# merlresearch/MC-PILCO

Hardware: NVIDIA B200
Metric: particle-steps/s (rollout fwd+bwd) (higher is better)
Workload: dtype f64

## Files before the change

### mc-pilco_b200/csrc/mcp_dgemm_tma.cu

```cuda
#include <cuda.h>

#include "mcp_dgemm.cuh"

namespace mcp {

constexpr int T_BM = 128, T_BN = 128, T_BK = 16, T_STAGES = 6, T_GROUP = 12;
constexpr int T_TILE_BYTES = T_BM * T_BK * 8;
constexpr int T_STAGE_BYTES = 2 * T_TILE_BYTES;
constexpr int T_CONSUMER_WARPS = 8;
constexpr int T_THREADS = 32 * T_CONSUMER_WARPS;
constexpr int T_LOOKAHEAD = T_STAGES - 2;
constexpr size_t T_SMEM_BYTES = (size_t)T_STAGES * T_STAGE_BYTES + 2 * T_STAGES * 8 + 1024;

__device__ __forceinline__ unsigned smem_u32(const void* p) { return (unsigned)__cvta_generic_to_shared(p); }
__device__ __forceinline__ void mbar_init(unsigned bar, unsigned count) {
  asm volatile("mbarrier.init.shared::cta.b64 [%0], %1;" ::"r"(bar), "r"(count));
}
__device__ __forceinline__ void mbar_expect_tx(unsigned bar, unsigned bytes) {
  asm volatile("mbarrier.arrive.expect_tx.shared::cta.b64 _, [%0], %1;" ::"r"(bar), "r"(bytes) : "memory");
}
__device__ __forceinline__ void mbar_arrive(unsigned bar) {
  asm volatile("mbarrier.arrive.shared::cta.b64 _, [%0];" ::"r"(bar) : "memory");
}
__device__ __forceinline__ void mbar_wait(unsigned bar, unsigned parity) {
  asm volatile(
      "{\n"
      ".reg .pred p;\n"
      "WAIT_%=:\n"
      "mbarrier.try_wait.parity.shared::cta.b64 p, [%0], %1;\n"
      "@p bra DONE_%=;\n"
      "bra WAIT_%=;\n"
      "DONE_%=:\n"
      "}\n" ::"r"(bar),
      "r"(parity)
      : "memory");
}
__device__ __forceinline__ void tma_load_2d(unsigned dst, const CUtensorMap* map, int c0, int c1, unsigned bar) {
  asm volatile("cp.async.bulk.tensor.2d.shared::cluster.global.mbarrier::complete_tx::bytes [%0], [%1, {%2, %3}], [%4];" ::"r"(dst),
               "l"(map), "r"(c0), "r"(c1), "r"(bar)
               : "memory");
}

template <bool TRIM>
__global__ void __launch_bounds__(T_THREADS, 1)
dgemm_tma_kernel(const __grid_constant__ CUtensorMap tmA, const __grid_constant__ CUtensorMap tmB, int M, int N, int K, double alpha,
                 double* __restrict__ C, int ldc, double beta, int tri, int kflags) {
  extern __shared__ unsigned char smem_raw[];
  const unsigned base = (smem_u32(smem_raw) + 1023u) & ~1023u;
  const unsigned char* tiles = smem_raw + (base - smem_u32(smem_raw));
  const unsigned bars = base + T_STAGES * T_STAGE_BYTES;
  const int warp = threadIdx.x >> 5, lane = threadIdx.x & 31;
  const int tiles_m = (M + T_BM - 1) / T_BM, tiles_n = (N + T_BN - 1) / T_BN;
  const int per_group = T_GROUP * tiles_n, group = blockIdx.x / per_group, first_m = group * T_GROUP;
  const int rows_here = min(tiles_m - first_m, T_GROUP), in_group = blockIdx.x - group * per_group;
  int mt = first_m + in_group % rows_here;
  if (TRIM && (kflags & KF_A_LOWER) && !(kflags & (KF_A_UPPER | KF_B_UPPER | KF_B_LOWER))) mt = tiles_m - 1 - mt;
  const int m0 = mt * T_BM;
  int nt = in_group / rows_here;
  if (TRIM && (kflags & KF_B_LOWER) && !(kflags & (KF_A_UPPER | KF_B_UPPER))) nt = tiles_n - 1 - nt;
  const int n0 = nt * T_BN;
  int kb = 0, ke = K;
  if (TRIM) {
    if (tri == 1 && n0 > m0 + T_BM - 1) return;
    if (kflags & KF_A_UPPER) kb = max(kb, m0);
    if (kflags & KF_B_UPPER) kb = max(kb, n0);
    if (kflags & KF_A_LOWER) ke = min(ke, m0 + T_BM);
    if (kflags & KF_B_LOWER) ke = min(ke, n0 + T_BN);
    kb = (kb / T_BK) * T_BK;
  }
  const int KT = ke > kb ? (ke - kb + T_BK - 1) / T_BK : 0;

  if (threadIdx.x == 0) {
#pragma unroll
    for (int s = 0; s < T_STAGES; s++) {
      mbar_init(bars + 8 * s, 1);
      mbar_init(bars + 8 * (T_STAGES + s), T_CONSUMER_WARPS);
    }
    asm volatile("fence.mbarrier_init.release.cluster;" ::: "memory");
  }
  __syncthreads();

  auto produce = [&](int kn) {
    const int s = kn % T_STAGES;
    if (kn >= T_STAGES) mbar_wait(bars + 8 * (T_STAGES + s), ((kn / T_STAGES) - 1) & 1);
    const unsigned full = bars + 8 * s, dst = base + s * T_STAGE_BYTES;
    mbar_expect_tx(full, T_STAGE_BYTES);
    tma_load_2d(dst, &tmA, kb + kn * T_BK, m0, full);
    tma_load_2d(dst + T_TILE_BYTES, &tmB, kb + kn * T_BK, n0, full);
  };
  if (threadIdx.x == 0) {
    asm volatile("prefetch.tensormap [%0];" ::"l"(&tmA) : "memory");
    asm volatile("prefetch.tensormap [%0];" ::"l"(&tmB) : "memory");
    for (int kn = 0; kn < T_LOOKAHEAD && kn < KT; kn++) produce(kn);
  }

  constexpr int MI = 4, NJ = 8;
  const int g = lane >> 2, q = lane & 3;
  const int wm0 = (warp & 3) * 32, wn0 = (warp >> 2) * 64;
  const unsigned kx = (unsigned)(g & 3) << 5;
  const unsigned laneE = ((unsigned)(q >> 1) << 4) | ((unsigned)(q & 1) << 3);
  const unsigned laneO = ((unsigned)((q >> 1) ^ 1) << 4) | ((unsigned)(q & 1) << 3);
  const unsigned aE = (unsigned)(wm0 + 2 * g) * 128u + laneE, aO = (unsigned)(wm0 + 2 * g + 1) * 128u + laneO;
  const unsigned bE = T_TILE_BYTES + (unsigned)(wn0 + 2 * g) * 128u + laneE, bO = T_TILE_BYTES + (unsigned)(wn0 + 2 * g + 1) * 128u + laneO;

  double acc[MI][NJ][2];
#pragma unroll
  for (int i = 0; i < MI; i++)
#pragma unroll
    for (int j = 0; j < NJ; j++) acc[i][j][0] = acc[i][j][1] = 0.0;

  for (int kt = 0; kt < KT; kt++) {
    const int s = kt % T_STAGES;
    if (threadIdx.x == 0 && kt + T_LOOKAHEAD < KT) produce(kt + T_LOOKAHEAD);
    mbar_wait(bars + 8 * s, (kt / T_STAGES) & 1);
    const unsigned char* st = tiles + s * T_STAGE_BYTES;
#pragma unroll
    for (int ks = 0; ks < T_BK / 4; ks++) {
      const unsigned ko = ((unsigned)(ks * 2) << 4) ^ kx;
      double a[MI], b[NJ];
#pragma unroll
      for (int i = 0; i < MI; i++) a[i] = *reinterpret_cast<const double*>(st + (((i & 1) ? aO : aE) + ko + (unsigned)(i >> 1) * 2048u));
#pragma unroll
      for (int j = 0; j < NJ; j++) b[j] = *reinterpret_cast<const double*>(st + (((j & 1) ? bO : bE) + ko + (unsigned)(j >> 1) * 2048u));
#pragma unroll
      for (int i = 0; i < MI; i++)
#pragma unroll
        for (int j = 0; j < NJ; j++) dmma884(acc[i][j][0], acc[i][j][1], a[i], b[j]);
    }
    __syncwarp();
    if (lane == 0) mbar_arrive(bars + 8 * (T_STAGES + s));
  }

#pragma unroll
  for (int i = 0; i < MI; i++) {
    const int r = m0 + wm0 + 16 * (i >> 1) + 2 * g + (i & 1);
    if (r >= M) continue;
#pragma unroll
    for (int jp = 0; jp < NJ / 2; jp++) {
      const int c = n0 + wn0 + 16 * jp + 4 * q;
      double* p = C + (size_t)r * ldc + c;
      double v0 = alpha * acc[i][2 * jp][0], v1 = alpha * acc[i][2 * jp + 1][0];
      double v2 = alpha * acc[i][2 * jp][1], v3 = alpha * acc[i][2 * jp + 1][1];
      if (TRIM && beta != 0.0) {
        if (c < N) v0 = fma(beta, p[0], v0);
        if (c + 1 < N) v1 = fma(beta, p[1], v1);
        if (c + 2 < N) v2 = fma(beta, p[2], v2);
        if (c + 3 < N) v3 = fma(beta, p[3], v3);
      }
      if (c + 3 < N) {
        *reinterpret_cast<double2*>(p) = make_double2(v0, v1);
        *reinterpret_cast<double2*>(p + 2) = make_double2(v2, v3);
      } else {
        if (c < N) p[0] = v0;
        if (c + 1 < N) p[1] = v1;
        if (c + 2 < N) p[2] = v2;
        if (c + 3 < N) p[3] = v3;
      }
    }
  }
}

typedef CUresult (*EncodeTiledFn)(CUtensorMap*, CUtensorMapDataType, cuuint32_t, void*, const cuuint64_t*, const cuuint64_t*,
                                  const cuuint32_t*, const cuuint32_t*, CUtensorMapInterleave, CUtensorMapSwizzle,
                                  CUtensorMapL2promotion, CUtensorMapFloatOOBfill);

static EncodeTiledFn encode_fn() {
  static EncodeTiledFn fn = nullptr;
  static bool tried = false;
  std::lock_guard<std::mutex> lock(init_mutex());
  if (!tried) {
    tried = true;
    void* p = nullptr;
    cudaDriverEntryPointQueryResult qres;
    if (cudaGetDriverEntryPoint("cuTensorMapEncodeTiled", &p, cudaEnableDefault, &qres) == cudaSuccess && qres == cudaDriverEntryPointSuccess)
      fn = (EncodeTiledFn)p;
  }
  return fn;
}

static int make_map(CUtensorMap* map, const double* ptr, int rows, int K, int ld) {
  EncodeTiledFn fn = encode_fn();
  if (!fn) {
    set_error("cuTensorMapEncodeTiled is not available from the CUDA driver");
    return MCP_E_CUDA;
  }
  cuuint64_t dims[2] = {(cuuint64_t)K, (cuuint64_t)rows};
  cuuint64_t strides[1] = {(cuuint64_t)ld * sizeof(double)};
  cuuint32_t box[2] = {(cuuint32_t)T_BK, (cuuint32_t)T_BM};
  cuuint32_t estr[2] = {1, 1};
  CUresult r = fn(map, CU_TENSOR_MAP_DATA_TYPE_FLOAT64, 2, (void*)ptr, dims, strides, box, estr, CU_TENSOR_MAP_INTERLEAVE_NONE,
                  CU_TENSOR_MAP_SWIZZLE_128B, CU_TENSOR_MAP_L2_PROMOTION_L2_256B, CU_TENSOR_MAP_FLOAT_OOB_FILL_NONE);
  if (r != CUDA_SUCCESS) {
    set_error("cuTensorMapEncodeTiled failed (%d) for a [%d x %d] matrix with ld %d", (int)r, rows, K, ld);
    return MCP_E_CUDA;
  }
  return MCP_OK;
}

bool dgemm_tma_usable(const double* A, int lda, const double* B, int ldb, const double* C, int ldc) {
  return ((uintptr_t)A % 16 == 0) && ((uintptr_t)B % 16 == 0) && ((uintptr_t)C % 16 == 0) && lda % 2 == 0 && ldb % 2 == 0 && ldc % 2 == 0 &&
         encode_fn() != nullptr;
}

template <bool TRIM>
static int launch_tma(int M, int N, int K, double alpha, const double* A, int lda, const double* B, int ldb, double beta, double* C, int ldc,
                      int tri, int kflags, cudaStream_t st) {
  static bool configured[MCP_MAX_DEVICES] = {};
  MCP_CUDA(ensure_dynamic_smem(configured, dgemm_tma_kernel<TRIM>, (int)T_SMEM_BYTES));
  CUtensorMap tmA, tmB;
  if (int e = make_map(&tmA, A, M, K, lda)) return e;
  if (int e = make_map(&tmB, B, N, K, ldb)) return e;
  dim3 grid((unsigned)cdiv(N, T_BN) * (unsigned)cdiv(M, T_BM));
  dgemm_tma_kernel<TRIM><<<grid, T_THREADS, T_SMEM_BYTES, st>>>(tmA, tmB, M, N, K, alpha, C, ldc, beta, tri, kflags);
  MCP_LAUNCH_CHECK();
  return MCP_OK;
}

int dgemm_nt_tma(int M, int N, int K, double alpha, const double* A, int lda, const double* B, int ldb, double* C, int ldc, cudaStream_t st) {
  if (M <= 0 || N <= 0) return MCP_OK;
  MCP_CHECK_ARG(dgemm_tma_usable(A, lda, B, ldb, C, ldc), "dgemm_nt_tma: operands must be 16-byte aligned with even leading dimensions");
  return launch_tma<false>(M, N, K, alpha, A, lda, B, ldb, 0.0, C, ldc, 0, 0, st);
}

int dgemm_nt_tma_trim(int M, int N, int K, double alpha, const double* A, int lda, const double* B, int ldb, double beta, double* C, int ldc,
                      int tri, int kflags, cudaStream_t st) {
  if (M <= 0 || N <= 0) return MCP_OK;
  MCP_CHECK_ARG(dgemm_tma_usable(A, lda, B, ldb, C, ldc), "dgemm_nt_tma_trim: operands must be 16-byte aligned with even leading dimensions");
  return launch_tma<true>(M, N, K, alpha, A, lda, B, ldb, beta, C, ldc, tri, kflags, st);
}

}
```

Baseline: 132,500.

## Make TMA DGEMM persistent and warp-specialized, splitting tail tiles into quarters

Turns the DGEMM into a persistent kernel whose grid is capped at the SM count. A dedicated producer warp issues TMA loads and uses setmaxnreg to hand its registers to eight consumer warps, which double-buffer their shared-memory fragment loads. When the last wave would leave SMs idle, the leftover 128x128 tiles are split into four 64x64 quarter tiles using extra tensor maps, to balance the final wave. The aim is to remove launch and wave-quantization waste and to overlap loads with DMMA compute, at the cost of more complex barrier phase tracking across tiles and three idle warps per CTA.

```diff
diff --git a/mc-pilco_b200/csrc/mcp_dgemm_tma.cu b/mc-pilco_b200/csrc/mcp_dgemm_tma.cu
--- a/mc-pilco_b200/csrc/mcp_dgemm_tma.cu
+++ b/mc-pilco_b200/csrc/mcp_dgemm_tma.cu
@@ -7,9 +7,10 @@
 constexpr int T_BM = 128, T_BN = 128, T_BK = 16, T_STAGES = 6, T_GROUP = 12;
 constexpr int T_TILE_BYTES = T_BM * T_BK * 8;
 constexpr int T_STAGE_BYTES = 2 * T_TILE_BYTES;
+constexpr int T_QUARTER_BYTES = T_STAGE_BYTES / 2;
 constexpr int T_CONSUMER_WARPS = 8;
-constexpr int T_THREADS = 32 * T_CONSUMER_WARPS;
-constexpr int T_LOOKAHEAD = T_STAGES - 2;
+constexpr int T_THREADS = 128 + 32 * T_CONSUMER_WARPS;
+constexpr int T_PRODUCER_REGS = 40, T_CONSUMER_REGS = 232;
 constexpr size_t T_SMEM_BYTES = (size_t)T_STAGES * T_STAGE_BYTES + 2 * T_STAGES * 8 + 1024;
 
 __device__ __forceinline__ unsigned smem_u32(const void* p) { return (unsigned)__cvta_generic_to_shared(p); }
@@ -40,63 +41,60 @@
                "l"(map), "r"(c0), "r"(c1), "r"(bar)
                : "memory");
 }
-
+__device__ __forceinline__ bool elect_one() {
+  unsigned pred;
+  asm volatile(
+      "{\n"
+      ".reg .pred p;\n"
+      "elect.sync _|p, 0xffffffff;\n"
+      "selp.u32 %0, 1, 0, p;\n"
+      "}\n"
+      : "=r"(pred));
+  return pred != 0;
+}
+
+struct TmaTile {
+  int m0, n0, kb, kt;
+  bool quarter;
+};
 template <bool TRIM>
-__global__ void __launch_bounds__(T_THREADS, 1)
-dgemm_tma_kernel(const __grid_constant__ CUtensorMap tmA, const __grid_constant__ CUtensorMap tmB, int M, int N, int K, double alpha,
-                 double* __restrict__ C, int ldc, double beta, int tri, int kflags) {
-  extern __shared__ unsigned char smem_raw[];
-  const unsigned base = (smem_u32(smem_raw) + 1023u) & ~1023u;
-  const unsigned char* tiles = smem_raw + (base - smem_u32(smem_raw));
-  const unsigned bars = base + T_STAGES * T_STAGE_BYTES;
-  const int warp = threadIdx.x >> 5, lane = threadIdx.x & 31;
+__device__ __forceinline__ bool tma_tile(int w, int M, int N, int K, int nfull, int tri, int kflags, TmaTile& t) {
   const int tiles_m = (M + T_BM - 1) / T_BM, tiles_n = (N + T_BN - 1) / T_BN;
-  const int per_group = T_GROUP * tiles_n, group = blockIdx.x / per_group, first_m = group * T_GROUP;
-  const int rows_here = min(tiles_m - first_m, T_GROUP), in_group = blockIdx.x - group * per_group;
+  const int tile = w < nfull ? w : nfull + ((w - nfull) >> 2);
+  const int per_group = T_GROUP * tiles_n, group = tile / per_group, first_m = group * T_GROUP;
+  const int rows_here = min(tiles_m - first_m, T_GROUP), in_group = tile - group * per_group;
   int mt = first_m + in_group % rows_here;
   if (TRIM && (kflags & KF_A_LOWER) && !(kflags & (KF_A_UPPER | KF_B_UPPER | KF_B_LOWER))) mt = tiles_m - 1 - mt;
-  const int m0 = mt * T_BM;
   int nt = in_group / rows_here;
   if (TRIM && (kflags & KF_B_LOWER) && !(kflags & (KF_A_UPPER | KF_B_UPPER))) nt = tiles_n - 1 - nt;
-  const int n0 = nt * T_BN;
+  t.m0 = mt * T_BM;
+  t.n0 = nt * T_BN;
+  t.quarter = w >= nfull;
+  if (t.quarter) {
+    const int qd = (w - nfull) & 3;
+    t.m0 += (qd & 1) * (T_BM / 2);
+    t.n0 += (qd >> 1) * (T_BN / 2);
+    if (t.m0 >= M || t.n0 >= N) return false;
+  }
   int kb = 0, ke = K;
   if (TRIM) {
-    if (tri == 1 && n0 > m0 + T_BM - 1) return;
-    if (kflags & KF_A_UPPER) kb = max(kb, m0);
-    if (kflags & KF_B_UPPER) kb = max(kb, n0);
-    if (kflags & KF_A_LOWER) ke = min(ke, m0 + T_BM);
-    if (kflags & KF_B_LOWER) ke = min(ke, n0 + T_BN);
+    if (tri == 1 && t.n0 > t.m0 + T_BM - 1) return false;
+    if (kflags & KF_A_UPPER) kb = max(kb, t.m0);
+    if (kflags & KF_B_UPPER) kb = max(kb, t.n0);
+    if (kflags & KF_A_LOWER) ke = min(ke, t.m0 + T_BM);
+    if (kflags & KF_B_LOWER) ke = min(ke, t.n0 + T_BN);
     kb = (kb / T_BK) * T_BK;
   }
-  const int KT = ke > kb ? (ke - kb + T_BK - 1) / T_BK : 0;
-
-  if (threadIdx.x == 0) {
-#pragma unroll
-    for (int s = 0; s < T_STAGES; s++) {
-      mbar_init(bars + 8 * s, 1);
-      mbar_init(bars + 8 * (T_STAGES + s), T_CONSUMER_WARPS);
-    }
-    asm volatile("fence.mbarrier_init.release.cluster;" ::: "memory");
-  }
-  __syncthreads();
-
-  auto produce = [&](int kn) {
-    const int s = kn % T_STAGES;
-    if (kn >= T_STAGES) mbar_wait(bars + 8 * (T_STAGES + s), ((kn / T_STAGES) - 1) & 1);
-    const unsigned full = bars + 8 * s, dst = base + s * T_STAGE_BYTES;
-    mbar_expect_tx(full, T_STAGE_BYTES);
-    tma_load_2d(dst, &tmA, kb + kn * T_BK, m0, full);
-    tma_load_2d(dst + T_TILE_BYTES, &tmB, kb + kn * T_BK, n0, full);
-  };
-  if (threadIdx.x == 0) {
-    asm volatile("prefetch.tensormap [%0];" ::"l"(&tmA) : "memory");
-    asm volatile("prefetch.tensormap [%0];" ::"l"(&tmB) : "memory");
-    for (int kn = 0; kn < T_LOOKAHEAD && kn < KT; kn++) produce(kn);
-  }
-
-  constexpr int MI = 4, NJ = 8;
+  t.kb = kb;
+  t.kt = ke > kb ? (ke - kb + T_BK - 1) / T_BK : 0;
+  return true;
+}
+
+template <int MI, int NJ, bool TRIM>
+__device__ __forceinline__ void consume_tile(const unsigned char* tiles, unsigned bars, int it, const TmaTile& t, int cw, int lane, int M,
+                                             int N, double alpha, double* __restrict__ C, int ldc, double beta) {
   const int g = lane >> 2, q = lane & 3;
-  const int wm0 = (warp & 3) * 32, wn0 = (warp >> 2) * 64;
+  const int wm0 = (cw & 3) * (8 * MI), wn0 = (cw >> 2) * (8 * NJ);
   const unsigned kx = (unsigned)(g & 3) << 5;
   const unsigned laneE = ((unsigned)(q >> 1) << 4) | ((unsigned)(q & 1) << 3);
   const unsigned laneO = ((unsigned)((q >> 1) ^ 1) << 4) | ((unsigned)(q & 1) << 3);
@@ -108,24 +106,36 @@
   for (int i = 0; i < MI; i++)
 #pragma unroll
     for (int j = 0; j < NJ; j++) acc[i][j][0] = acc[i][j][1] = 0.0;
-
-  for (int kt = 0; kt < KT; kt++) {
-    const int s = kt % T_STAGES;
-    if (threadIdx.x == 0 && kt + T_LOOKAHEAD < KT) produce(kt + T_LOOKAHEAD);
-    mbar_wait(bars + 8 * s, (kt / T_STAGES) & 1);
+  double a[2][MI], b[2][NJ];
+  auto load = [&](int set, const unsigned char* st, int ks) {
+    const unsigned ko = ((unsigned)(ks * 2) << 4) ^ kx;
+#pragma unroll
+    for (int i = 0; i < MI; i++) a[set][i] = *reinterpret_cast<const double*>(st + (((i & 1) ? aO : aE) + ko + (unsigned)(i >> 1) * 2048u));
+#pragma unroll
+    for (int j = 0; j < NJ; j++) b[set][j] = *reinterpret_cast<const double*>(st + (((j & 1) ? bO : bE) + ko + (unsigned)(j >> 1) * 2048u));
+  };
+
+  if (t.kt > 0) {
+    const int s = it % T_STAGES;
+    mbar_wait(bars + 8 * s, (it / T_STAGES) & 1);
+    load(0, tiles + s * T_STAGE_BYTES, 0);
+  }
+  for (int kt = 0; kt < t.kt; kt++) {
+    const int s = (it + kt) % T_STAGES;
     const unsigned char* st = tiles + s * T_STAGE_BYTES;
 #pragma unroll
     for (int ks = 0; ks < T_BK / 4; ks++) {
-      const unsigned ko = ((unsigned)(ks * 2) << 4) ^ kx;
-      double a[MI], b[NJ];
-#pragma unroll
-      for (int i = 0; i < MI; i++) a[i] = *reinterpret_cast<const double*>(st + (((i & 1) ? aO : aE) + ko + (unsigned)(i >> 1) * 2048u));
-#pragma unroll
-      for (int j = 0; j < NJ; j++) b[j] = *reinterpret_cast<const double*>(st + (((j & 1) ? bO : bE) + ko + (unsigned)(j >> 1) * 2048u));
+      if (ks + 1 < T_BK / 4) {
+        load((ks + 1) & 1, st, ks + 1);
+      } else if (kt + 1 < t.kt) {
+        const int n = it + kt + 1, s1 = n % T_STAGES;
+        mbar_wait(bars + 8 * s1, (n / T_STAGES) & 1);
+        load(0, tiles + s1 * T_STAGE_BYTES, 0);
+      }
 #pragma unroll
       for (int i = 0; i < MI; i++)
 #pragma unroll
-        for (int j = 0; j < NJ; j++) dmma884(acc[i][j][0], acc[i][j][1], a[i], b[j]);
+        for (int j = 0; j < NJ; j++) dmma884(acc[i][j][0], acc[i][j][1], a[ks & 1][i], b[ks & 1][j]);
     }
     __syncwarp();
     if (lane == 0) mbar_arrive(bars + 8 * (T_STAGES + s));
@@ -133,11 +143,11 @@
 
 #pragma unroll
   for (int i = 0; i < MI; i++) {
-    const int r = m0 + wm0 + 16 * (i >> 1) + 2 * g + (i & 1);
+    const int r = t.m0 + wm0 + 16 * (i >> 1) + 2 * g + (i & 1);
     if (r >= M) continue;
 #pragma unroll
     for (int jp = 0; jp < NJ / 2; jp++) {
-      const int c = n0 + wn0 + 16 * jp + 4 * q;
+      const int c = t.n0 + wn0 + 16 * jp + 4 * q;
       double* p = C + (size_t)r * ldc + c;
       double v0 = alpha * acc[i][2 * jp][0], v1 = alpha * acc[i][2 * jp + 1][0];
       double v2 = alpha * acc[i][2 * jp][1], v3 = alpha * acc[i][2 * jp + 1][1];
@@ -160,6 +170,71 @@
   }
 }
 
+template <bool TRIM>
+__global__ void __launch_bounds__(T_THREADS, 1)
+dgemm_tma_kernel(const __grid_constant__ CUtensorMap tmA, const __grid_constant__ CUtensorMap tmB, const __grid_constant__ CUtensorMap tmA64,
+                 const __grid_constant__ CUtensorMap tmB64, int M, int N, int K, int nfull, int items, double alpha, double* __restrict__ C,
+                 int ldc, double beta, int tri, int kflags) {
+  extern __shared__ unsigned char smem_raw[];
+  const unsigned base = (smem_u32(smem_raw) + 1023u) & ~1023u;
+  const unsigned char* tiles = smem_raw + (base - smem_u32(smem_raw));
+  const unsigned bars = base + T_STAGES * T_STAGE_BYTES;
+  const int warp = threadIdx.x >> 5, lane = threadIdx.x & 31;
+
+  if (threadIdx.x == 0) {
+#pragma unroll
+    for (int s = 0; s < T_STAGES; s++) {
+      mbar_init(bars + 8 * s, 1);
+      mbar_init(bars + 8 * (T_STAGES + s), T_CONSUMER_WARPS);
+    }
+    asm volatile("fence.mbarrier_init.release.cluster;" ::: "memory");
+  }
+  __syncthreads();
+
+  if (warp < 4) {
+    asm volatile("setmaxnreg.dec.sync.aligned.u32 %0;" ::"n"(T_PRODUCER_REGS));
+    if (warp != 0) return;
+    const bool leader = elect_one();
+    if (leader) {
+      asm volatile("prefetch.tensormap [%0];" ::"l"(&tmA) : "memory");
+      asm volatile("prefetch.tensormap [%0];" ::"l"(&tmB) : "memory");
+    }
+    int it = 0;
+    for (int w = blockIdx.x; w < items; w += gridDim.x) {
+      TmaTile t;
+      if (!tma_tile<TRIM>(w, M, N, K, nfull, tri, kflags, t)) continue;
+      const CUtensorMap* ma = t.quarter ? &tmA64 : &tmA;
+      const CUtensorMap* mb = t.quarter ? &tmB64 : &tmB;
+      const unsigned bytes = t.quarter ? T_QUARTER_BYTES : T_STAGE_BYTES;
+      for (int kt = 0; kt < t.kt; kt++, it++) {
+        const int s = it % T_STAGES;
+        if (it >= T_STAGES) mbar_wait(bars + 8 * (T_STAGES + s), ((it / T_STAGES) - 1) & 1);
+        if (leader) {
+          const unsigned full = bars + 8 * s, dst = base + s * T_STAGE_BYTES;
+          mbar_expect_tx(full, bytes);
+          tma_load_2d(dst, ma, t.kb + kt * T_BK, t.m0, full);
+          tma_load_2d(dst + T_TILE_BYTES, mb, t.kb + kt * T_BK, t.n0, full);
+        }
+        __syncwarp();
+      }
+    }
+    return;
+  }
+
+  asm volatile("setmaxnreg.inc.sync.aligned.u32 %0;" ::"n"(T_CONSUMER_REGS));
+  const int cw = warp - 4;
+  int it = 0;
+  for (int w = blockIdx.x; w < items; w += gridDim.x) {
+    TmaTile t;
+    if (!tma_tile<TRIM>(w, M, N, K, nfull, tri, kflags, t)) continue;
+    if (!TRIM && t.quarter)
+      consume_tile<2, 4, TRIM>(tiles, bars, it, t, cw, lane, M, N, alpha, C, ldc, beta);
+    else
+      consume_tile<4, 8, TRIM>(tiles, bars, it, t, cw, lane, M, N, alpha, C, ldc, beta);
+    it += t.kt;
+  }
+}
+
 typedef CUresult (*EncodeTiledFn)(CUtensorMap*, CUtensorMapDataType, cuuint32_t, void*, const cuuint64_t*, const cuuint64_t*,
                                   const cuuint32_t*, const cuuint32_t*, CUtensorMapInterleave, CUtensorMapSwizzle,
                                   CUtensorMapL2promotion, CUtensorMapFloatOOBfill);
@@ -178,7 +253,7 @@
   return fn;
 }
 
-static int make_map(CUtensorMap* map, const double* ptr, int rows, int K, int ld) {
+static int make_map(CUtensorMap* map, const double* ptr, int rows, int K, int ld, int box_rows) {
   EncodeTiledFn fn = encode_fn();
   if (!fn) {
     set_error("cuTensorMapEncodeTiled is not available from the CUDA driver");
@@ -186,7 +261,7 @@
   }
   cuuint64_t dims[2] = {(cuuint64_t)K, (cuuint64_t)rows};
   cuuint64_t strides[1] = {(cuuint64_t)ld * sizeof(double)};
-  cuuint32_t box[2] = {(cuuint32_t)T_BK, (cuuint32_t)T_BM};
+  cuuint32_t box[2] = {(cuuint32_t)T_BK, (cuuint32_t)box_rows};
   cuuint32_t estr[2] = {1, 1};
   CUresult r = fn(map, CU_TENSOR_MAP_DATA_TYPE_FLOAT64, 2, (void*)ptr, dims, strides, box, estr, CU_TENSOR_MAP_INTERLEAVE_NONE,
                   CU_TENSOR_MAP_SWIZZLE_128B, CU_TENSOR_MAP_L2_PROMOTION_L2_256B, CU_TENSOR_MAP_FLOAT_OOB_FILL_NONE);
@@ -207,11 +282,25 @@
                       int tri, int kflags, cudaStream_t st) {
   static bool configured[MCP_MAX_DEVICES] = {};
   MCP_CUDA(ensure_dynamic_smem(configured, dgemm_tma_kernel<TRIM>, (int)T_SMEM_BYTES));
-  CUtensorMap tmA, tmB;
-  if (int e = make_map(&tmA, A, M, K, lda)) return e;
-  if (int e = make_map(&tmB, B, N, K, ldb)) return e;
-  dim3 grid((unsigned)cdiv(N, T_BN) * (unsigned)cdiv(M, T_BM));
-  dgemm_tma_kernel<TRIM><<<grid, T_THREADS, T_SMEM_BYTES, st>>>(tmA, tmB, M, N, K, alpha, C, ldc, beta, tri, kflags);
+  CUtensorMap tmA, tmB, tmA64, tmB64;
+  if (int e = make_map(&tmA, A, M, K, lda, T_BM)) return e;
+  if (int e = make_map(&tmB, B, N, K, ldb, T_BN)) return e;
+  if (int e = make_map(&tmA64, A, M, K, lda, T_BM / 2)) return e;
+  if (int e = make_map(&tmB64, B, N, K, ldb, T_BN / 2)) return e;
+  const int tiles = cdiv(N, T_BN) * cdiv(M, T_BM);
+  int nfull = tiles, items = tiles, grid = tiles;
+  if (!TRIM) {
+    int dev = 0, sms = 0;
+    MCP_CUDA(cudaGetDevice(&dev));
+    MCP_CUDA(cudaDeviceGetAttribute(&sms, cudaDevAttrMultiProcessorCount, dev));
+    const int rem = tiles % sms;
+    if (rem > 0 && 4 * rem <= 3 * sms) {
+      nfull = tiles - rem;
+      items = nfull + 4 * rem;
+    }
+    grid = items < sms ? items : sms;
+  }
+  dgemm_tma_kernel<TRIM><<<grid, T_THREADS, T_SMEM_BYTES, st>>>(tmA, tmB, tmA64, tmB64, M, N, K, nfull, items, alpha, C, ldc, beta, tri, kflags);
   MCP_LAUNCH_CHECK();
   return MCP_OK;
 }
```

New measurement: 133,700 (median of 6 runs). Within noise of the previous version (+0.9%).
